# Icelk/fractal-renderer

Measured on AMD Instinct MI355X. Metric: pixel_iterations_per_sec, higher is better.
Workload: dtype f64

## Files before the change

fractal-renderer_amd/_native.py:

```python
import ctypes as C
import os

PKG_DIR = os.path.dirname(os.path.abspath(__file__))
LIB_PATH = os.path.join(PKG_DIR, "libfractal_hip.so")

FR_OK, FR_ERR_INVALID_ARGUMENT, FR_ERR_BUFFER_TOO_SMALL, FR_ERR_NO_DEVICE, FR_ERR_HIP = 0, 1, 2, 3, 4
STATUS_NAMES = {
    1: "FR_ERR_INVALID_ARGUMENT",
    2: "FR_ERR_BUFFER_TOO_SMALL",
    3: "FR_ERR_NO_DEVICE",
    4: "FR_ERR_HIP",
    5: "FR_ERR_UNSUPPORTED_ALGO",
}


class FractalHipError(RuntimeError):
    def __init__(self, code, message):
        super().__init__("%s: %s" % (STATUS_NAMES.get(code, "fr_status %d" % code), message))
        self.code = code


class Imaginary(C.Structure):

    _fields_ = [("re", C.c_double), ("im", C.c_double)]
# ... 158 lines not shown
    "fr_escape_rows": (C.c_int, [C.POINTER(fr_config), C.c_int, C.c_uint32, C.c_uint32, C.c_void_p, C.c_void_p]),
    "fr_render_rows_dd": (
        C.c_int, [C.POINTER(fr_config), C.POINTER(Imaginary), C.c_uint32, C.c_uint32, C.c_int, C.c_void_p, C.c_size_t]),
    "fr_render_rows_dd_device": (
        C.c_int,
        [C.POINTER(fr_config), C.POINTER(Imaginary), C.c_uint32, C.c_uint32, C.c_int, C.c_void_p, C.c_size_t, C.c_void_p],
    ),
    "fr_escape_rows_dd": (
        C.c_int, [C.POINTER(fr_config), C.POINTER(Imaginary), C.c_uint32, C.c_uint32, C.c_void_p, C.c_void_p]),
    "fr_render_rows_pt": (
        C.c_int, [C.POINTER(fr_config), C.POINTER(Imaginary), C.c_uint32, C.c_uint32, C.c_int, C.c_void_p, C.c_size_t]),
    "fr_render_rows_pt_device": (
        C.c_int,
        [C.POINTER(fr_config), C.POINTER(Imaginary), C.c_uint32, C.c_uint32, C.c_int, C.c_void_p, C.c_size_t, C.c_void_p],
    ),
    "fr_escape_rows_pt": (
        C.c_int, [C.POINTER(fr_config), C.POINTER(Imaginary), C.c_uint32, C.c_uint32, C.c_void_p, C.c_void_p]),
    "fr_debug_reference_orbit": (
        C.c_int, [C.POINTER(fr_config), C.POINTER(Imaginary), C.c_int, C.c_void_p, C.c_size_t, C.POINTER(C.c_uint32)]),
    "fr_colour_rgb8": (C.c_int, [C.POINTER(fr_config), C.c_void_p, C.c_void_p, C.c_size_t, C.c_void_p, C.c_size_t]),
    "fr_colour_rgb8_device": (
        C.c_int, [C.POINTER(fr_config), C.c_void_p, C.c_void_p, C.c_size_t, C.c_void_p, C.c_size_t, C.c_void_p]),
    "fr_count_iterations": (
        C.c_int,
        [C.POINTER(fr_config), C.c_int, C.c_uint32, C.c_uint32, C.c_uint32, C.c_uint32, C.POINTER(C.c_uint64),
         C.POINTER(C.c_uint64)],
    ),
    "fr_set_profiling": (C.c_int, [C.c_int]),
    "fr_last_kernel_ms": (C.c_int, [C.POINTER(C.c_float)]),
    "fr_set_tile": (C.c_int, [C.c_int]),
    "fr_set_loop_mode": (C.c_int, [C.c_int]),
    "fr_debug_loop_plan": (C.c_int, [C.POINTER(fr_config), C.c_int, C.POINTER(C.c_uint32), C.POINTER(C.c_double),
                                     C.POINTER(C.c_uint32)]),
    "fr_set_palette": (C.c_int, [C.c_int]),
    "fr_set_cycle_shortcut": (C.c_int, [C.c_int]),
    "fr_set_refill_policy": (C.c_int, [C.c_int, C.c_int]),
    "fr_debug_math": (C.c_int, [C.c_int, C.c_void_p, C.c_void_p, C.c_size_t]),
    "fr_debug_set_queue_trace": (C.c_int, [C.c_void_p]),
    "fr_debug_set_two_pass_capacity": (C.c_int, [C.c_uint32]),
}

_lib = None


def load():
    global _lib
    if _lib is not None:
        return _lib
    if not os.path.exists(LIB_PATH):
        raise ImportError(
            "%s is missing — build it first (python -c 'import __graft_entry__ as g; g.build()'); "
            "this package has no CPU fallback" % LIB_PATH
        )
    lib = C.CDLL(LIB_PATH)
    for name, (restype, argtypes) in PROTOTYPES.items():
        fn = getattr(lib, name)
        fn.restype = restype
        fn.argtypes = argtypes
    _lib = lib
    return lib


def check(rc):
    if rc != FR_OK:
        msg = load().fr_last_error()
        raise FractalHipError(rc, msg.decode() if msg else "")
# ... 1 lines not shown
```

fractal-renderer_amd/csrc/fr_api.hip:

```cpp
#include <hip/hip_runtime.h>

#include <atomic>
#include <cmath>
#include <cstddef>
#include <cstdint>
#include <cstdio>
#include <cstdlib>
#include <cstring>
#include <mutex>
#include <shared_mutex>
#include <string>
#include <vector>

#include "fr_ctx.h"

static_assert(sizeof(fr_config) == 104 && offsetof(fr_config, limit) == 16 && offsetof(fr_config, inside) == 72 &&
                  offsetof(fr_config, primary_color) == 74 && offsetof(fr_config, color_weight) == 80 &&
                  offsetof(fr_config, julia_set) == 88,
              "fr_config must stay the #[repr(C)] image of calc::Config");
static_assert(sizeof(fr_render_opts) == 32, "fr_render_opts is part of the ABI");

namespace fr {

namespace {

thread_local std::string tl_error;
thread_local Profiling tl_prof;
std::atomic<bool> g_process_exiting{false};

std::shared_mutex g_life;
std::mutex g_primary_mu;
Ctx g_primary;
bool g_primary_inited = false;

std::atomic<int> g_tile{0};
std::atomic<int> g_palette_enabled{1};
std::atomic<int> g_cycle_shortcut{0};
std::atomic<int> g_refill_minrun{-1}, g_refill_quit16{-1};
std::atomic<int> g_loop_mode{-1};
std::atomic<int> g_colour_filter{1};
std::atomic<unsigned long long *> g_queue_trace{nullptr};
std::atomic<uint32_t> g_two_pass_list_entries{0};

bool valid_tile(int tile) {
    switch (tile) {
    case 0: case 1: case 2: case 4: case 8: case 9: case 10: case 11: case 12: case 13: case 14: case 15: case 16: case 6401: case 3202: case 1604: case 808:
        return true;
    default:
        return false;
    }
}

}

int fail(int code, const char *what) {
    tl_error = what;
    return code;
}
int fail(int code, const std::string &what) {
    tl_error = what;
    return code;
}

int fail_hip(hipError_t e, const char *what) {
    char buf[512];
    snprintf(buf, sizeof buf, "%s: %s (%s)", what, hipGetErrorString(e), hipGetErrorName(e));
    tl_error = buf;
    (void)hipGetLastError();
    return (e == hipErrorNoDevice || e == hipErrorInvalidDevice) ? FR_ERR_NO_DEVICE : FR_ERR_HIP;
}

const std::string &last_error() { return tl_error; }

LifeShared::LifeShared() { g_life.lock_shared(); }
LifeShared::~LifeShared() { g_life.unlock_shared(); }
// ... 421 lines not shown
    {
        static const int dbg_want = getenv("FR_DEBUG_QUEUE_WANT") ? atoi(getenv("FR_DEBUG_QUEUE_WANT")) : 0;
        static const int dbg_minrun = getenv("FR_DEBUG_QUEUE_MINRUN") ? atoi(getenv("FR_DEBUG_QUEUE_MINRUN")) : -1;
        if (dbg_want > 0 && dbg_want <= 64) p.queue_want = (uint32_t)dbg_want;
        if (dbg_minrun >= 0) p.queue_minrun = (uint32_t)dbg_minrun;
    }
    {
        static const int dbg_ablate = getenv("FR_DEBUG_ABLATE") ? atoi(getenv("FR_DEBUG_ABLATE")) : 0;
        p.debug_ablate = (uint32_t)dbg_ablate & 3u;
    }
    p.cycle_shortcut = (o.cycle_shortcut && cfg->iterations < (1u << 30)) ? 1u : 0u;
    p.filt_k = n != 0 ? cfg->exposure / (double)n : 0.0;
    const bool filter_ok = o.colour_filter && cfg->smooth && n != 0 && std::isfinite(cfg->exposure) &&
                           std::fabs(p.filt_k) <= 1e100 && cfg->stable_limit >= 0.0;
    p.colour_filter = filter_ok ? 1u : 0u;
    const double ak = std::fabs(p.filt_k);
    p.colour_filter32 = (filter_ok && o.colour_filter == 1 && n < (1u << 24) && ak >= 0x1p-60 && ak <= 0x1p60) ? 1u : 0u;
    p.filt_k32 = (float)p.filt_k;
    p.filt_c32 = p.colour_filter32 ? std::nextafterf((float)(ak * FR_NU_BRACKET * (1.0 + 0x1p-9)), INFINITY) : 0.0f;
    for (int k = 0; k < 3; k++) {
        p.filt_d[k] = p.prim_f[k] * ak * FR_NU_BRACKET * (1.0 + 0x1p-20);
        p.filt_d32[k] = p.colour_filter32 ? std::nextafterf((float)(p.prim_f[k] * ak * FR_NU_BRACKET * (1.0 + 0x1p-10)), INFINITY) : 0.0f;
        p.prim32[k] = (float)p.prim[k];
    }
    const double lo = std::fmax(cfg->stable_limit, 2.0) * (1.0 + 0x1p-20);
    p.filt_lo32 = (p.colour_filter32 && lo < 1e30) ? std::nextafterf((float)lo, INFINITY) : INFINITY;
}

static double host_coord(double coord, double max, double offset, double pos, double scale) {
    return ((coord / max) - offset) / scale + pos;
}

constexpr uint32_t kSpecQuiet = 16;

void plan_loop(const fr_config *cfg, int precision, const Opts &o, fr_kparams &p) {
    p.loop_mode = 0;
    p.skip_t = 0.0;
    p.loop_spec = 0;
    const bool no_spec = o.loop_mode == 5;
    const int forced = no_spec ? -1 : o.loop_mode;
    if (cfg->algo != FR_ALGO_MANDELBROT && cfg->algo != FR_ALGO_JULIA) return;
    if (p.ncols == 0 || p.nrows == 0) return;
    const bool f32 = precision == FR_PRECISION_F32;
    const double range_hi = f32 ? 0x1p30 : 0x1p400;
    const double slack = f32 ? 1.0 + 0x1p-18 : 1.0 + 0x1p-30;
    double lim2;
    if (f32) {
        const float lf = (float)cfg->limit;
        lim2 = (double)(lf * lf);
    } else {
        lim2 = cfg->limit * cfg->limit;
    }
    auto mag = [f32](double v) { return std::fabs(f32 ? (double)(float)v : v); };
    const double w = (double)cfg->width, h = (double)cfg->height;
    const uint64_t x_last = (uint64_t)p.x_first + (uint64_t)(p.ncols - 1) * p.x_stride;
    const uint32_t r_last = p.nrows - 1;
    const uint64_t y_last = (uint64_t)p.y_first + (uint64_t)(r_last / p.block_rows) * p.y_stride + r_last % p.block_rows;
    if (x_last > 0xFFFFFFFFull || y_last > 0xFFFFFFFFull) return;
    auto nmax = [](double a, double b) { return (a != a || b != b) ? NAN : std::fmax(a, b); };
    double smax = 0.0;
    for (double x : {(double)p.x_first, (double)x_last})
        smax = nmax(smax, mag(host_coord(x, h, (w / h) / 2.0, cfg->pos.re, cfg->scale.re)));
    for (double y : {(double)p.y_first, (double)y_last})
        smax = nmax(smax, mag(host_coord(y, h, 0.5, cfg->pos.im, cfg->scale.im)));
    const double cmax = cfg->algo == FR_ALGO_JULIA ? nmax(mag(cfg->julia_set.re), mag(cfg->julia_set.im)) : smax;
    if (!no_spec && lim2 >= 16.0 && lim2 <= (f32 ? 0x1p100 : 0x1p1000) && cmax <= lim2 / 8.0 && smax <= (f32 ? 0x1p120 : 0x1p1000)) {
        static const int dbg = getenv("FR_DEBUG_SPEC_QUIET") ? atoi(getenv("FR_DEBUG_SPEC_QUIET")) : 0;
        p.loop_spec = dbg > 0 ? (uint32_t)dbg : kSpecQuiet;
    }
    if (forced == 0) return;
    if (!(std::fabs(cfg->limit) <= range_hi)) return;
    if (!(cmax <= range_hi)) return;
    for (int m : {4, 2}) {
        if (forced > 0 && forced != m) continue;
        double d = lim2;
        for (int j = 1; j < m && d > 0.0; j++) d = std::sqrt(d / (2.0 * slack)) - cmax;
        double t = d * (1.0 - 0x1p-20);
        if (f32) {
            float tf = (float)t;
            if ((double)tf > t) tf = std::nextafterf(tf, 0.0f);
            t = (double)tf;
        }
        if (t >= 4.5 || (forced == m && t > 0.0)) {
            p.loop_mode = (uint32_t)m;
            p.skip_t = t;
            if (!(t < lim2)) p.loop_spec = 0;
            return;
        }
    }
}

static int check_rows(const fr_config *cfg, uint32_t y0, uint32_t y1) {
    if (!cfg) return fail(FR_ERR_INVALID_ARGUMENT, "cfg is NULL");
    if (y0 > y1) return fail(FR_ERR_INVALID_ARGUMENT, "y0 > y1");
    if (y1 > cfg->height) return fail(FR_ERR_INVALID_ARGUMENT, "y1 > height");
    return FR_OK;
}

int check_precision(int precision) {
    if (precision == FR_PRECISION_DD)
        return fail(FR_ERR_INVALID_ARGUMENT, "FR_PRECISION_DD is single-device only: the row renders, fr_pixel_p, fr_escape_rows(_dd) "
                                             "and fr_count_iterations take it");
    if (precision == FR_PRECISION_PT)
        return fail(FR_ERR_INVALID_ARGUMENT, "FR_PRECISION_PT is single-device only: the row renders, fr_pixel_p, fr_escape_rows(_pt) "
                                             "and fr_count_iterations take it");
    if (precision != FR_PRECISION_F64 && precision != FR_PRECISION_F32)
        return fail(FR_ERR_INVALID_ARGUMENT, "precision must be FR_PRECISION_F64 or FR_PRECISION_F32");
    return FR_OK;
}

static int check_deep(const fr_config *cfg, const fr_imaginary *pos_lo, const char *name) {
    if (!cfg) return fail(FR_ERR_INVALID_ARGUMENT, "cfg is NULL");
    const std::string n(name);
    const double lo_re = pos_lo ? pos_lo->re : 0.0, lo_im = pos_lo ? pos_lo->im : 0.0;
    const double fields[] = {cfg->limit,    cfg->stable_limit, cfg->pos.re,       cfg->pos.im,       cfg->scale.re, cfg->scale.im,
                             cfg->exposure, cfg->color_weight, cfg->julia_set.re, cfg->julia_set.im, lo_re,         lo_im};
    for (double v : fields)
        if (!std::isfinite(v)) return fail(FR_ERR_INVALID_ARGUMENT, n + ": every field of the view must be finite");
    if (!(cfg->limit > 0.0 && cfg->limit <= 0x1p500))
// ... 995 lines not shown
}

int fr_debug_view_choice(const fr_config *cfg, int precision, uint32_t y0, uint32_t y1, int *state, int *choice,
                         uint32_t *strip_tiles) {
    if (!cfg || !state || !choice || !strip_tiles) return fail(FR_ERR_INVALID_ARGUMENT, "NULL argument");
    int rc = check_rows(cfg, y0, y1);
    if (rc == FR_OK) rc = check_precision(precision);
    if (rc != FR_OK) return rc;
    LifeShared ls;
    Ctx *ctx;
    rc = primary(&ctx);
    if (rc != FR_OK) return rc;
    fr_kparams p;
    fill_params(cfg, default_opts(), p);
    p.nrows = y1 - y0;
    p.y_first = y0;
    p.block_rows = p.nrows ? p.nrows : 1;
    p.y_stride = 0;
    const uint64_t key = view_key(cfg, p, precision);
    *state = 0, *choice = -1, *strip_tiles = 0;
    std::lock_guard<std::mutex> lk(ctx->sample_mu);
    for (int k = 0; k < Ctx::kViewChoices; k++) {
        const Ctx::ViewChoice &v = ctx->view_choices[k];
        if (v.key != key || v.state == 0) continue;
        *state = v.state;
        if (v.state == 1 && __atomic_load_n(ctx->sample_result + 8 * k + 7, __ATOMIC_ACQUIRE) == key) *state = 3;
        *choice = v.two_pass;
        *strip_tiles = v.strip_tiles;
        break;
    }
    return FR_OK;
}

int fr_debug_set_queue_trace(void *d_trace) {
    g_queue_trace.store(static_cast<unsigned long long *>(d_trace));
    return FR_OK;
}

int fr_debug_set_two_pass_capacity(uint32_t entries_per_list) {
    g_two_pass_list_entries.store(entries_per_list);
    return FR_OK;
}

int fr_debug_math(int which, const double *in, double *out, size_t n) {
    if (n == 0) return FR_OK;
    if (!in || !out) return fail(FR_ERR_INVALID_ARGUMENT, "NULL array");
    LifeShared ls;
    Ctx *ctx;
    int rc = primary(&ctx);
    if (rc != FR_OK) return rc;
    std::lock_guard<std::mutex> lk(ctx->mu);
    rc = ctx->reserve(ctx->z, 2 * n * sizeof(double));
    if (rc != FR_OK) return rc;
    double *d_in = static_cast<double *>(ctx->z.ptr), *d_out = d_in + n;
    if (which == 4) {
        if (n < 2) return fail(FR_ERR_INVALID_ARGUMENT, "which == 4 needs n >= 2");
        HIP_TRY(fr_launch_nu_scan((uint32_t)in[0], (uint32_t)in[1], d_out, ctx->stream));
        HIP_TRY(hipMemcpyAsync(out, d_out, sizeof(double), hipMemcpyDeviceToHost, ctx->stream));
        HIP_TRY(hipStreamSynchronize(ctx->stream));
        return FR_OK;
    }
    if (which == 6) {
        if (n < 2) return fail(FR_ERR_INVALID_ARGUMENT, "which == 6 needs n >= 2");
        HIP_TRY(fr_launch_cast_scan((uint32_t)in[0], (uint32_t)in[1], d_out, ctx->stream));
        unsigned long long bad = 0;
        HIP_TRY(hipMemcpyAsync(&bad, d_out, sizeof bad, hipMemcpyDeviceToHost, ctx->stream));
// ... 13 lines not shown
```

fractal-renderer_amd/csrc/fr_kernels.h:

```cpp
#ifndef FR_KERNELS_H
#define FR_KERNELS_H

#include <hip/hip_runtime.h>
#include <stdint.h>

struct fr_kparams {
    uint32_t algo;
    uint32_t width, height;
    uint32_t iterations;
    double limit, stable_limit;
    double pos_re, pos_im, scale_re, scale_im;
    double exposure;
    double julia_re, julia_im;
    uint32_t inside, smooth;
    uint32_t prim[3], sec[3];
    double prim_f[3], sec_f[3];
    double iterations_f64, inv_iterations;
    uint32_t ncols, nrows;
    uint32_t x_first, x_stride;
    uint32_t block_rows, y_first, y_stride;
    uint32_t out_in_place;
    uint32_t out_rgba;
    uint32_t loop_mode;
    double skip_t;
    uint32_t loop_spec;
    uint32_t first_no_spec;
    const uint32_t *palette;
    uint32_t palette_entries;
    uint32_t refill_minrun, refill_quit16;
    uint32_t queue_minrun, queue_want;
    uint32_t cycle_shortcut;
    uint32_t colour_filter;
    uint32_t *work_counter;
    double filt_k;
    double filt_d[3];
    uint32_t colour_filter32;
    float filt_k32;
    float filt_c32;
    float filt_d32[3];
    float prim32[3];
    float filt_lo32;
    uint32_t first_cap;
    uint32_t first_keep;
    uint32_t two_pass_cap;
    uint32_t first_only;
    uint32_t second_v1;
    uint32_t first_one_band;
    uint32_t strip_tiles;
    uint32_t debug_ablate;
    uint32_t surv_sub_capacity;
    void *surv_z;
    uint32_t *surv_pos;
    uint32_t *surv_cnt;
    void *surv_c;
    uint32_t *surv_counts;
};

constexpr uint32_t FR_SURV_QUEUES = 64;
// ... 61 lines not shown
```

fractal-renderer_amd/csrc/fr_kernels.hip:

```cpp
#include "fr_kernels.h"

#include <cmath>

#include <cstdlib>

#include "fr_math.h"

namespace {

#include "fr_colour.h"

constexpr int kWaves = 4;


#define FR_ORBIT_STEP(SFX, TAG)                    \
    "v_add_" SFX " %[t], %[r2], -%[i2]\n"          \
    "v_add_" SFX " %[x], %[re], %[re]\n"           \
    "v_add_" SFX " %[re], %[t], %[cre]\n"          \
    "v_mul_" SFX " %[x], %[x], %[im]\n"            \
    "v_add_" SFX " %[im], %[x], %[cim]\n"          \
    "v_mul_" SFX " %[r2], %[re], %[re]\n"          \
    "v_mul_" SFX " %[i2], %[im], %[im]\n"          \
    "v_add_" SFX " %[t], %[r2], %[i2]\n"           \
    "s_mov_b64 %[sprev], exec\n"                   \
// ... 167 lines not shown
    "v_mul_" SFX " %[q], %[X], %[Y]\n"             \
    "v_fma_" SFX " %[X], %[t], 0.5, %[c2re]\n"     \
    "v_add_" SFX " %[Y], %[q], %[c2im]\n"          \
    "v_mul_" SFX " %[A], %[X], %[X]\n"             \
    "v_mul_" SFX " %[B], %[Y], %[Y]\n"

#define FR_SC_IT_R(SFX, S, D)                              \
    "v_add_" SFX " %[t], %[A" S "], -%[B" S "]\n"          \
    "v_mul_" SFX " %[q], %[X" S "], %[Y" S "]\n"           \
    "v_fma_" SFX " %[X" D "], %[t], 0.5, %[c2re]\n"        \
    "v_add_" SFX " %[Y" D "], %[q], %[c2im]\n"             \
    "v_mul_" SFX " %[A" D "], %[X" D "], %[X" D "]\n"      \
    "v_mul_" SFX " %[B" D "], %[Y" D "], %[Y" D "]\n"
#define FR_SC_IT_R5(SFX, S) FR_SC_IT_R(SFX, S, S) FR_SC_IT_R(SFX, S, S) FR_SC_IT_R(SFX, S, S) FR_SC_IT_R(SFX, S, S) FR_SC_IT_R(SFX, S, S)

#define FR_SC_SPEC_ENTRY(MSTR)                                                     \
    "s_cmp_lt_u32 %[si], %[sspec]\n"                                               \
    "s_cbranch_scc1 .Lfast_%=\n"                                                   \
    "s_cmp_lt_u32 %[si], %[n]\n"                                                   \
    "s_cbranch_scc0 .Ldone_%=\n"                                                   \
    "s_sub_u32 %[stmp], %[n], %[si]\n"                                             \
    "s_cmp_ge_u32 %[stmp], " MSTR "\n"                                             \
    "s_cbranch_scc1 .Lspec_%=\n"                                                   \
    "s_mov_b32 %[sspec], %[n]\n"                                                   \
    "s_branch .Lfast_%=\n"
#define FR_SC_NOSPEC_ENTRY                                                         \
    "s_cmp_lt_u32 %[si], %[n]\n"                                                   \
    "s_cbranch_scc1 .Lfast_%=\n"                                                   \
    "s_branch .Ldone_%=\n"
#define FR_SC_SPEC_ARM                                                             \
    "s_add_u32 %[sspec], %[si], %[specq]\n"                                        \
    "s_cselect_b32 %[sspec], -1, %[sspec]\n"                                       \
    "s_min_u32 %[sspec], %[sspec], %[n]\n"
#define FR_SC_SPEC_BODY(SFX, MOV, MSTR, REST)                                      \
    ".Lspec_%=:\n" FR_SC_IT_R(SFX, "", "1") REST(SFX, "1")                         \
    "v_add_" SFX " %[t], %[A1], %[B1]\n"                                           \
    "v_cmp_nge_" SFX " vcc, %[t4lim], %[t]\n"                                      \
    "s_cbranch_vccnz .LrbA_%=\n"                                                   \
    "s_add_u32 %[si], %[si], " MSTR "\n"                                           \
    "s_sub_u32 %[stmp], %[n], %[si]\n"                                             \
    "s_cmp_ge_u32 %[stmp], " MSTR "\n"                                             \
    "s_cbranch_scc0 .LexA_%=\n"                                                    \
    FR_SC_IT_R(SFX, "1", "") REST(SFX, "")                                         \
    "v_add_" SFX " %[t], %[A], %[B]\n"                                             \
    "v_cmp_nge_" SFX " vcc, %[t4lim], %[t]\n"                                      \
    "s_cbranch_vccnz .LrbB_%=\n"                                                   \
    "s_add_u32 %[si], %[si], " MSTR "\n"                                           \
    "s_sub_u32 %[stmp], %[n], %[si]\n"                                             \
    "s_cmp_ge_u32 %[stmp], " MSTR "\n"                                             \
    "s_cbranch_scc1 .Lspec_%=\n"                                                   \
    "s_branch .Lspecout_%=\n"                                                      \
    ".LexA_%=:\n"                                                                  \
    MOV " %[X], %[X1]\n" MOV " %[Y], %[Y1]\n" MOV " %[A], %[A1]\n" MOV " %[B], %[B1]\n" \
    ".Lspecout_%=:\n"                                                              \
    "s_mov_b32 %[sspec], %[n]\n"                                                   \
    "s_cmp_lt_u32 %[si], %[n]\n"                                                   \
    "s_cbranch_scc1 .Lfast_%=\n"                                                   \
    "s_branch .Ldone_%=\n"                                                         \
    ".LrbB_%=:\n"                                                                  \
    MOV " %[X], %[X1]\n" MOV " %[Y], %[Y1]\n" MOV " %[A], %[A1]\n" MOV " %[B], %[B1]\n" \
    ".LrbA_%=:\n"                                                                  \
    "s_lshl_b32 %[specq], %[specq], 1\n"                                           \
    "s_min_u32 %[specq], %[specq], 0x8000\n"                                       \
    FR_SC_SPEC_ARM                                                                 \
    "s_branch .Lfast_%=\n"

#define FR_SC_CHECKED_STEP(SFX, TAG)               \
    FR_SC_IT(SFX)                                  \
    "v_add_" SFX " %[t], %[A], %[B]\n"             \
    "s_mov_b64 %[sprev], exec\n"                   \
    "v_cmpx_nlt_" SFX " %[lim4], %[t]\n"           \
    "s_xor_b64 %[sdiff], %[sprev], exec\n"         \
    "s_cbranch_scc1 .Lrec" TAG "_%=\n"             \
    ".Lcont" TAG "_%=:\n"

#define FR_SC_ASM(SFX, MSTR, FAST_ITS, SLOW_STEPS, SLOW_RECORDS, CYC_F, CYC_S, CYC_H, SP_INIT, SP_ARM, SP_ENTRY, SP_BODY)  \
    "s_mov_b64 %[sorig], exec\n"                                                   \
    "v_mov_b32 %[it], %[n]\n"                                                      \
    "s_mov_b32 %[si], 0\n"                                                         \
    SP_INIT                                                                        \
    "s_cbranch_execz .Ldone_%=\n"                                                  \
    "v_add_" SFX " %[t], %[A], %[B]\n"                                                         \
    "s_and_b32 %[nrem], %[n], " MSTR "-1\n"                                        \
    "s_cbranch_scc0 .Lmodesel_%=\n"                                                \
    ".Lrem_%=:\n" FR_SC_CHECKED_STEP(SFX, "R")                                     \
    "s_add_u32 %[si], %[si], 1\n"                                                  \
    "s_cmp_lt_u32 %[si], %[nrem]\n"                                                \
    "s_cbranch_scc1 .Lrem_%=\n"                                                    \
    ".Lmodesel_%=:\n"                                                              \
    "s_cmp_lt_u32 %[si], %[n]\n"                                                   \
    "s_cbranch_scc0 .Ldone_%=\n"                                                   \
    "v_cmp_lt_" SFX " vcc, %[t4lim], %[t]\n"                                       \
    "s_cbranch_vccnz .Lslow_%=\n"                                                  \
    ".Lfast_%=:\n" FAST_ITS                                                        \
// ... 53 lines not shown
    "v_mov_b32 %[vsaved], %[si]\n"                 \
    "s_lshl_b32 %[snext], %[snext], 1\n"           \
    "s_branch .Lsavecont" TAG "_%=\n"

#define FR_SC_CYC_HANDLER(TAG)                     \
    ".Lcyc" TAG "_%=:\n"                           \
    "s_or_b32 %[stmp], %[si], 0x80000000\n"        \
    "s_mov_b64 %[sprev], exec\n"                   \
    "s_mov_b64 exec, %[scyc]\n"                    \
    "v_mov_b32 %[it], %[stmp]\n"                   \
    "s_andn2_b64 exec, %[sprev], %[scyc]\n"        \
    "s_cbranch_execz .Ldone_%=\n"                  \
    "s_bcnt1_i32_b64 %[scnt], exec\n"              \
    "s_cmp_gt_u32 %[scnt], %[thr]\n"               \
    "s_cbranch_scc1 .Lcyccont" TAG "_%=\n"         \
    "s_cmp_lt_u32 %[si], %[minrun]\n"              \
    "s_cbranch_scc1 .Lcyccont" TAG "_%=\n"         \
    "s_branch .Ldone_%=\n"

#define FR_SC_ASM_M4_(SFX, CYC_F, CYC_S, CYC_H, SP_INIT, SP_ARM, SP_ENTRY, SP_BODY)                 \
    FR_SC_ASM(SFX, "4", FR_SC_IT(SFX) FR_SC_IT(SFX) FR_SC_IT(SFX) FR_SC_IT(SFX),                    \
              FR_SC_CHECKED_STEP(SFX, "A") FR_SC_CHECKED_STEP(SFX, "B") FR_SC_CHECKED_STEP(SFX, "C") \
                  FR_SC_CHECKED_STEP(SFX, "D"),                                                     \
              FR_ORBIT_RECORD("A", "0") FR_ORBIT_RECORD("B", "1") FR_ORBIT_RECORD("C", "2")         \
                  FR_ORBIT_RECORD("D", "3"),                                                        \
              CYC_F, CYC_S, CYC_H, SP_INIT, SP_ARM, SP_ENTRY, SP_BODY)
#define FR_SC_ASM_M2_(SFX, CYC_F, CYC_S, CYC_H)                                            \
    FR_SC_ASM(SFX, "2", FR_SC_IT(SFX) FR_SC_IT(SFX),                                        \
              FR_SC_CHECKED_STEP(SFX, "A") FR_SC_CHECKED_STEP(SFX, "B"),                    \
              FR_ORBIT_RECORD("A", "0") FR_ORBIT_RECORD("B", "1"), CYC_F, CYC_S, CYC_H, "", "", FR_SC_NOSPEC_ENTRY, "")
#define FR_SC_ASM_M4(SFX) FR_SC_ASM_M4_(SFX, "", "", "", "", "", FR_SC_NOSPEC_ENTRY, "")
#define FR_SC_ASM_M2(SFX) FR_SC_ASM_M2_(SFX, "", "", "")
#define FR_SC_ASM_M4_SPEC(SFX, MOV)                                                                 \
    FR_SC_ASM_M4_(SFX, "", "", "", "s_min_u32 %[sspec], %[specq], %[n]\n", FR_SC_SPEC_ARM, FR_SC_SPEC_ENTRY(FR_SPEC_MSTR), \
                  FR_SC_SPEC_BODY(SFX, MOV, FR_SPEC_MSTR, FR_SC_SPEC_REST))
#define FR_SC_CYC_HANDLERS(MOV) \
    FR_SC_CYC_HANDLER("F") FR_SC_CYC_HANDLER("S") FR_SC_CYC_SAVE(MOV, "F") FR_SC_CYC_SAVE(MOV, "S")
#define FR_SC_ASM_M4_CYC(SFX, EQ, MOV) \
    FR_SC_ASM_M4_(SFX, FR_SC_CYC_CHECK(EQ, "F"), FR_SC_CYC_CHECK(EQ, "S"), FR_SC_CYC_HANDLERS(MOV), "", "", FR_SC_NOSPEC_ENTRY, "")
#define FR_SC_ASM_M2_CYC(SFX, EQ, MOV) \
    FR_SC_ASM_M2_(SFX, FR_SC_CYC_CHECK(EQ, "F"), FR_SC_CYC_CHECK(EQ, "S"), FR_SC_CYC_HANDLERS(MOV))

template <typename T>
struct ScalableRange;
template <>
struct ScalableRange<double> {
    static constexpr double lo = 0x1p-300, hi = 0x1p400;
};
template <>
struct ScalableRange<float> {
    static constexpr float lo = 0x1p-30f, hi = 0x1p30f;
};

template <typename T>
__device__ __forceinline__ bool lane_is_scalable(T re0, T im0, T cre, T cim) {
    constexpr T lo = ScalableRange<T>::lo, hi = ScalableRange<T>::hi;
    auto c_ok = [=](T v) { return __builtin_fabs(v) >= lo && __builtin_fabs(v) <= hi; };
    auto s_ok = [=](T v) { return v == (T)0 || c_ok(v); };
    return c_ok(cre) && c_ok(cim) && s_ok(re0) && s_ok(im0);
}

template <typename T, int M, bool CYC>
__device__ __forceinline__ uint32_t orbit_scaled_run(uint32_t iterations, T &X, T &Y, T &A, T &B, T c2re, T c2im,
                                                     T squared, T skip_t, EpisodeCtl ctl, uint32_t &completed,
                                                     T *pXs = nullptr, T *pYs = nullptr,
                                                     uint32_t *saved_index = nullptr, uint32_t spec_quiet = 0u) {
    uint32_t it;
    T t, q;
    T X1, Y1, A1, B1;
    uint32_t sspec;
    uint32_t specq = __builtin_amdgcn_readfirstlane(spec_quiet ? spec_quiet : 0xFFFFFFFFu);
    T Xs = CYC ? *pXs : T(0), Ys = CYC ? *pYs : T(0);
    uint32_t vsaved = 0xFFFFFFFFu;
    uint32_t snext = 32u;
    unsigned long long sorig, sprev, sdiff, scyc;
    uint32_t si, stmp, nrem, scnt;
    const uint32_t n = __builtin_amdgcn_readfirstlane(iterations);
    const uint32_t thr = __builtin_amdgcn_readfirstlane(ctl.thr), minrun = __builtin_amdgcn_readfirstlane(ctl.minrun);
    const T lim4_v = (T)4 * squared, t4_v = (T)4 * skip_t;
#define FR_SC_OUTPUTS                                                                                           \
    [X] "+v"(X), [Y] "+v"(Y), [A] "+v"(A), [B] "+v"(B), [it] "=&v"(it), [t] "=&v"(t), [q] "=&v"(q),             \
        [sorig] "=&s"(sorig), [sprev] "=&s"(sprev), [sdiff] "=&s"(sdiff), [si] "=&s"(si), [stmp] "=&s"(stmp),   \
        [nrem] "=&s"(nrem), [scnt] "=&s"(scnt)
#define FR_SC_INPUTS                                                                                            \
    [c2re] "v"(c2re), [c2im] "v"(c2im), [lim4] "s"(lim4), [t4lim] "s"(t4lim), [n] "s"(n), [thr] "s"(thr),       \
        [minrun] "s"(minrun)
#define FR_SC_OPERANDS : FR_SC_OUTPUTS : FR_SC_INPUTS : "vcc", "scc"
#define FR_SC_OPERANDS_SPEC                                                                                     \
    : FR_SC_OUTPUTS, [X1] "=&v"(X1), [Y1] "=&v"(Y1), [A1] "=&v"(A1), [B1] "=&v"(B1), [sspec] "=&s"(sspec),      \
      [specq] "+&s"(specq)                                                                                      \
    : FR_SC_INPUTS                                                                                              \
    : "vcc", "scc"
#define FR_SC_OPERANDS_CYC                                                                                      \
    : FR_SC_OUTPUTS, [scyc] "=&s"(scyc), [Xs] "+v"(Xs), [Ys] "+v"(Ys), [vsaved] "+v"(vsaved), [snext] "+s"(snext) \
    : FR_SC_INPUTS                                                                                              \
    : "vcc", "scc"
    if constexpr (sizeof(T) == 8) {
        const uint64_t lb = fr_bits_of(lim4_v), tb = fr_bits_of(t4_v);
        const uint64_t lim4 = (uint64_t)(uint32_t)__builtin_amdgcn_readfirstlane((uint32_t)lb) |
                              ((uint64_t)(uint32_t)__builtin_amdgcn_readfirstlane((uint32_t)(lb >> 32)) << 32);
        const uint64_t t4lim = (uint64_t)(uint32_t)__builtin_amdgcn_readfirstlane((uint32_t)tb) |
                               ((uint64_t)(uint32_t)__builtin_amdgcn_readfirstlane((uint32_t)(tb >> 32)) << 32);
        if constexpr (M == 4 && CYC)
            asm volatile(FR_SC_ASM_M4_CYC("f64", "v_cmp_eq_u64", "v_mov_b64") FR_SC_OPERANDS_CYC);
        else if constexpr (M == 4)
            asm volatile(FR_SC_ASM_M4_SPEC("f64", "v_mov_b64") FR_SC_OPERANDS_SPEC);
        else if constexpr (CYC)
            asm volatile(FR_SC_ASM_M2_CYC("f64", "v_cmp_eq_u64", "v_mov_b64") FR_SC_OPERANDS_CYC);
        else
            asm volatile(FR_SC_ASM_M2("f64") FR_SC_OPERANDS);
    } else {
        const uint32_t lim4 = __builtin_amdgcn_readfirstlane(__builtin_bit_cast(uint32_t, lim4_v));
        const uint32_t t4lim = __builtin_amdgcn_readfirstlane(__builtin_bit_cast(uint32_t, t4_v));
        if constexpr (M == 4 && CYC)
            asm volatile(FR_SC_ASM_M4_CYC("f32", "v_cmp_eq_u32", "v_mov_b32") FR_SC_OPERANDS_CYC);
        else if constexpr (M == 4)
            asm volatile(FR_SC_ASM_M4_SPEC("f32", "v_mov_b32") FR_SC_OPERANDS_SPEC);
        else if constexpr (CYC)
            asm volatile(FR_SC_ASM_M2_CYC("f32", "v_cmp_eq_u32", "v_mov_b32") FR_SC_OPERANDS_CYC);
        else
            asm volatile(FR_SC_ASM_M2("f32") FR_SC_OPERANDS);
    }
    (void)scyc;
    (void)snext;
    (void)X1, (void)Y1, (void)A1, (void)B1, (void)sspec, (void)specq;
    if constexpr (CYC) {
        *pXs = Xs;
        *pYs = Ys;
        *saved_index = vsaved;
    }
    completed = si;
    return it;
}

template <typename T, int M>
__device__ __forceinline__ uint32_t orbit_scaled(uint32_t iterations, T &re, T &im, T cre, T cim, T squared,
                                                 T skip_t, T &r2, T &i2, uint32_t spec_quiet = 0u) {
    T X = re + re, Y = im + im, A = X * X, B = Y * Y;
    uint32_t completed;
    const uint32_t it = orbit_scaled_run<T, M, false>(iterations, X, Y, A, B, cre + cre, cim + cim, squared, skip_t,
                                               EpisodeCtl{0, 0}, completed, nullptr, nullptr, nullptr, spec_quiet);
    re = X * (T)0.5;
    im = Y * (T)0.5;
    r2 = re * re;
    i2 = im * im;
    return it;
}

template <typename T>
__device__ __forceinline__ uint32_t orbit_auto(uint32_t loop_mode, uint32_t iterations, T &re, T &im, T cre, T cim,
                                               T squared, T skip_t, T &r2, T &i2, int strip_scalable = -1,
                                               uint32_t spec_quiet = 0u) {
    if (loop_mode != 0 && strip_scalable != 0) {
        bool all_ok = strip_scalable == 1;
        if (strip_scalable < 0) all_ok = __ballot(!lane_is_scalable<T>(re, im, cre, cim)) == 0ull;
        if (all_ok) {
            if (loop_mode == 4) return orbit_scaled<T, 4>(iterations, re, im, cre, cim, squared, skip_t, r2, i2, spec_quiet);
            return orbit_scaled<T, 2>(iterations, re, im, cre, cim, squared, skip_t, r2, i2);
        }
    }
    return orbit<T>(iterations, re, im, cre, cim, squared, r2, i2, spec_quiet);
}

__device__ __forceinline__ double coord_to_space(double coord, double max, double offset, double pos,
                                                 double scale) {
    return ((coord / max) - offset) / scale + pos;
}

__device__ __forceinline__ void store_pixel(uint32_t ncols, uint32_t out_rgba, uint8_t *base, uint32_t row, uint32_t col,
                                            const uint8_t rgb[3]) {
    const uint64_t k = (uint64_t)row * ncols + col;
    if (out_rgba) {
        reinterpret_cast<uint32_t *>(base)[k] =
            (uint32_t)rgb[0] | ((uint32_t)rgb[1] << 8) | ((uint32_t)rgb[2] << 16) | 0xFF000000u;
    } else {
        uint8_t *o = base + 3ull * k;
        o[0] = rgb[0];
        o[1] = rgb[1];
        o[2] = rgb[2];
    }
}
__device__ __forceinline__ void store_pixel(const fr_kparams &p, uint8_t *base, uint32_t row, uint32_t col, const uint8_t rgb[3]) {
    store_pixel(p.ncols, p.out_rgba, base, row, col, rgb);
}

typedef const __attribute__((address_space(4))) fr_kparams *KArgs;
#define FR_COLD_PARAMS(NAME)                                                          \
    KArgs NAME = (KArgs)__builtin_amdgcn_kernarg_segment_ptr();  \
    asm volatile("" : "+s"(NAME))

// ... 20 lines not shown

__device__ __forceinline__ void store_packed(uint8_t *base, uint32_t off, uint32_t packed, uint32_t bpp) {
    if (bpp == 4u) {
        const uint32_t v = packed | 0xFF000000u;
        asm volatile("s_nop 4\n\tglobal_store_dword %0, %1, %2" : : "v"(off), "v"(v), "s"(base) : "memory");
    } else {
        asm volatile("s_nop 4\n\tglobal_store_short %0, %1, %2\n\tglobal_store_byte_d16_hi %0, %1, %2 offset:2" : : "v"(off), "v"(packed), "s"(base) : "memory");
    }
}

struct TileOut {
    uint8_t *base;
    uint32_t lane_off, bpp;
    bool narrow, fast_colour;
};

template <typename T>
__device__ __forceinline__ uint32_t colour_packed(bool valid, bool fast_colour, T re, T im, T r2, T i2, uint32_t iters,
                                                  const double *lds_tab, const uint32_t *palette) {
    uint32_t packed = 0;
    unsigned long long todo = ballot64(valid);
    if (fast_colour) {
        Filter32 f;
        {
            FR_COLD_PARAMS(kp);
            f.lo = kp->filt_lo32, f.k = kp->filt_k32, f.c = kp->filt_c32;
            f.p0 = kp->prim32[0], f.p1 = kp->prim32[2], f.p2 = kp->prim32[1];
        }
        float d32;
        if constexpr (sizeof(T) == 8)
            d32 = (float)(r2 + i2);
        else
            d32 = r2 + i2;
        uint32_t pk;
        const bool decided = colour_fast32(f, d32, (float)(iters + 1u), pk);
        const bool ok = valid && d32 >= f.lo && d32 <= 0x1.ffffep119f && decided;
        packed = ok ? pk : 0u;
        todo &= ~ballot64(ok);
    }
    if (todo != 0ull) {
        bool inside_done = false;
        if (lane_in(todo)) {
            double dist;
            if constexpr (sizeof(T) == 8) {
                dist = (double)(r2 + i2);
            } else {
                const double zre = (double)re, zim = (double)im;
                dist = zre * zre + zim * zim;
            }
            FR_COLD_PARAMS(kp);
            inside_done = !(dist > kp->stable_limit);
            if (inside_done && kp->inside)
                packed = sat_u8_dev(kp->sec_f[0] * dist) | (sat_u8_dev(kp->sec_f[2] * dist) << 8) | (sat_u8_dev(kp->sec_f[1] * dist) << 16);
        }
        todo &= ~ballot64(inside_done);
    }
    if (todo != 0ull) {
        if (lane_in(todo)) {
            FR_COLD_PARAMS(kp);
            const ColourConsts cc = make_colour_consts(*kp);
            uint8_t rgb[3];
            colour_pixel<T>(cc, re, im, r2, i2, iters, lds_tab, palette, rgb);
            packed = (uint32_t)rgb[0] | ((uint32_t)rgb[1] << 8) | ((uint32_t)rgb[2] << 16);
        }
    }
    return packed;
}

template <typename T, int MODE>
__device__ __forceinline__ void render_pixel(const fr_kparams &p, const fr_kout &out, const double *s_tab,
                                             const uint32_t *s_pal, double sre, double sim, bool valid,
                                             uint32_t cx, uint32_t r, uint32_t lane, uint32_t r_out,
                                             int strip_scalable = -1, const TileOut *to = nullptr) {
    double zre = 0.0, zim = 0.0;
    T tre = 0, tim = 0, tr2 = 0, ti2 = 0;
    uint32_t iters = 0;
    const bool escape_algo = p.algo == 0  || p.algo == 2 ;
    if (valid && escape_algo) {
        const double cre = p.algo == 0 ? sre : p.julia_re;
        const double cim = p.algo == 0 ? sim : p.julia_im;
        if constexpr (sizeof(T) == 8) {
            tre = sre;
            tim = sim;
            iters = orbit_auto<double>(p.loop_mode, p.iterations, tre, tim, cre, cim, p.limit * p.limit, p.skip_t,
                                       tr2, ti2, strip_scalable, p.loop_spec);
            zre = tre;
            zim = tim;
        } else {
            tre = (float)sre, tim = (float)sim;
            const float lim = (float)p.limit;
            iters = orbit_auto<float>(p.loop_mode, p.iterations, tre, tim, (float)cre, (float)cim, lim * lim,
                                      (float)p.skip_t, tr2, ti2, strip_scalable, p.loop_spec);
            zre = (double)tre;
            zim = (double)tim;
        }
    }

    if constexpr (MODE == FR_OUT_RGB) {
        if (to != nullptr) {
            uint32_t packed = 0;
            if (escape_algo) packed = colour_packed<T>(valid, to->fast_colour, tre, tim, tr2, ti2, iters, s_tab, s_pal);
            if (valid) {
                if (to->narrow) {
                    store_packed(to->base, to->lane_off, packed, to->bpp);
                } else {
                    const uint8_t rgb[3] = {(uint8_t)packed, (uint8_t)(packed >> 8), (uint8_t)(packed >> 16)};
                    store_pixel(p, out.rgb, r_out, cx, rgb);
                }
            }
        } else if (valid) {
            uint8_t rgb[3] = {0, 0, 0};
            if (escape_algo) {
                const ColourConsts cc = make_colour_consts(p);
                colour_pixel<T>(cc, tre, tim, tr2, ti2, iters, s_tab, s_pal, rgb);
            }
            store_pixel(p, out.rgb, r_out, cx, rgb);
        }
    } else if constexpr (MODE == FR_OUT_ESCAPE) {
        if (valid) {
            const uint64_t k = (uint64_t)r * p.ncols + cx;
            if (out.z) {
                out.z[2 * k] = zre;
                out.z[2 * k + 1] = zim;
            }
            if (out.iters) out.iters[k] = iters;
// ... 1005 lines not shown
            const uint32_t cx = tile0 * 8u + ccol, r = row0 + crow;
            if (cx < p.ncols && r < p.nrows) {
                const T zre = (T)sre, zim = (T)sim;
                const T cre = julia ? (T)p.julia_re : zre, cim = julia ? (T)p.julia_im : zim;
                if constexpr (FORM == 0) {
                    a0 = zre, a1 = zim, a2 = zre * zre, a3 = zim * zim, c0 = cre, c1 = cim;
                } else {
                    a0 = zre + zre, a1 = zim + zim, a2 = a0 * a0, a3 = a1 * a1, c0 = cre + cre, c1 = cim + cim;
                }
                if constexpr (CYC) xs = ys = cycle_none<T>(), saved_at = 0;
                px = cx, py = r, pout = sout;
                done = 0;
                busy = true;
            }
        }
        const uint32_t nfree = (uint32_t)__builtin_popcountll(free_mask);
        next = next + nfree < P ? next + nfree : P;
        const unsigned long long busy_mask = __ballot(busy);
        if (busy_mask == 0ull) {
            if (next >= P) break;
            continue;
        }

        const uint32_t n = wave_min_u32(busy ? iterations - done : 0xFFFFFFFFu);
        const uint32_t nbusy = (uint32_t)__builtin_popcountll(busy_mask);
        EpisodeCtl ctl{0u, 0u};
        if (next < P) ctl = EpisodeCtl{nbusy - (nbusy * p.refill_quit16 + 15) / 16, p.refill_minrun};
        uint32_t it = 0, completed = 0, saved_index = 0xFFFFFFFFu;
        if (busy) {
            if constexpr (FORM == 0)
                it = orbit_run<T>(n, a0, a1, c0, c1, squared, a2, a3, ctl, completed, p.loop_spec);
            else
                it = orbit_scaled_run<T, FORM, CYC>(n, a0, a1, a2, a3, c0, c1, squared, skip_t, ctl, completed, &xs, &ys,
                                                    &saved_index, p.loop_spec);
        }
        if (busy) {
            bool cycled = false;
            if constexpr (CYC) cycled = (it & 0x80000000u) != 0u;
            const bool escaped = !cycled && it < completed;
            const uint32_t before = done;
            if constexpr (CYC) {
                if (saved_index != 0xFFFFFFFFu) saved_at = before + saved_index;
            }
            if (cycled) {
                const uint32_t k = it & 0x7FFFFFFFu;
                const uint32_t d = before + k - saved_at;
                const uint32_t remaining = iterations - (before + k);
                done = iterations - remaining % d;
                xs = ys = cycle_none<T>();
            } else {
                done += completed;
            }
            if (escaped || done == iterations) {
                const uint32_t iters = escaped ? before + it : iterations;
                T fre, fim, fr2, fi2;
                if constexpr (FORM == 0) {
                    fre = a0, fim = a1, fr2 = a2, fi2 = a3;
                } else {
                    fre = a0 * (T)0.5, fim = a1 * (T)0.5;
                    fr2 = fre * fre, fi2 = fim * fim;
                }
                const double zre = (double)fre, zim = (double)fim;
                const double dist = sizeof(T) == 8 ? (double)(fr2 + fi2) : zre * zre + zim * zim;
                if constexpr (MODE == FR_OUT_RGB) {
                    uint8_t rgb[3];
                    colour_of(cc, dist, iters, s_tab, s_pal, rgb);
                    store_pixel(p, out.rgb, pout, px, rgb);
// ... 1475 lines not shown
```

include/fractal_hip.h:

```cpp
#ifndef FRACTAL_HIP_H
#define FRACTAL_HIP_H

#include <stddef.h>
#include <stdint.h>

#ifdef __cplusplus
extern "C" {
#endif

#define FR_ABI_VERSION 3

typedef enum fr_status {
    FR_OK = 0,
    FR_ERR_INVALID_ARGUMENT = 1,
    FR_ERR_BUFFER_TOO_SMALL = 2,
    FR_ERR_NO_DEVICE = 3,
    FR_ERR_HIP = 4,
    FR_ERR_UNSUPPORTED_ALGO = 5
} fr_status;

typedef enum fr_algo {
    FR_ALGO_MANDELBROT = 0,
    FR_ALGO_BARNSLEY_FERN = 1,
    FR_ALGO_JULIA = 2
// ... 166 lines not shown
int fr_escape_rows(const fr_config *cfg, int precision, uint32_t y0, uint32_t y1, double *z_re_im,
                   uint32_t *iters);

int fr_colour_rgb8(const fr_config *cfg, const double *z_re_im, const uint32_t *iters, size_t n, uint8_t *out,
                   size_t out_len);
int fr_colour_rgb8_device(const fr_config *cfg, const void *d_z_re_im, const void *d_iters, size_t n, void *d_out,
                          size_t out_len, void *hip_stream);


int fr_count_iterations(const fr_config *cfg, int precision, uint32_t y0, uint32_t y1, uint32_t sx,
                        uint32_t sy, uint64_t *total, uint64_t *pixels);

int fr_set_profiling(int enabled);
int fr_last_kernel_ms(float *ms);
int fr_last_kernel_name(char *buf, size_t buf_len);

int fr_set_tile(int tile);

int fr_set_dispatch_sampling(int enabled);
int fr_debug_sample_view(const fr_config *cfg, int precision, double out[8]);
int fr_debug_view_choice(const fr_config *cfg, int precision, uint32_t y0, uint32_t y1, int *state, int *choice,
                         uint32_t *strip_tiles);

int fr_set_refill_policy(int minrun, int quit16);

int fr_set_cycle_shortcut(int enabled);

int fr_set_palette(int enabled);

int fr_set_colour_filter(int enabled);

int fr_set_loop_mode(int mode);
int fr_debug_loop_plan(const fr_config *cfg, int precision, uint32_t *loop_mode, double *skip_t, uint32_t *spec_quiet);

int fr_debug_math(int which, const double *in, double *out, size_t n);
int fr_debug_set_queue_trace(void *d_trace);
int fr_debug_set_two_pass_capacity(uint32_t entries_per_list);

#ifdef __cplusplus
}
#endif
#endif
```

Before: 5312 billion.

## Grow speculative escape-check blocks geometrically up to a capped length

The speculative Mandelbrot/Julia inner loop checked for escape every fixed block of iterations. It now doubles the block length after each block without an escape, up to a cap (default 128, with a debug setter). On rollback the cap is reset to the base block. Fewer escape checks and branches run per iteration in long non-escaping stretches, at the cost of more rolled-back iterations when a lane escapes late in a long block. The colour filter is also gated on a wave ballot so fast-colour work is skipped when no lane is outside.

```diff
diff --git a/fractal-renderer_amd/_native.py b/fractal-renderer_amd/_native.py
--- a/fractal-renderer_amd/_native.py
+++ b/fractal-renderer_amd/_native.py
@@ -214,6 +214,8 @@
     "fr_set_loop_mode": (C.c_int, [C.c_int]),
     "fr_debug_loop_plan": (C.c_int, [C.POINTER(fr_config), C.c_int, C.POINTER(C.c_uint32), C.POINTER(C.c_double),
                                      C.POINTER(C.c_uint32)]),
+    "fr_debug_set_spec_maxlen": (C.c_int, [C.c_uint32]),
+    "fr_debug_spec_maxlen": (C.c_int, [C.POINTER(fr_config), C.c_int, C.POINTER(C.c_uint32)]),
     "fr_set_palette": (C.c_int, [C.c_int]),
     "fr_set_cycle_shortcut": (C.c_int, [C.c_int]),
     "fr_set_refill_policy": (C.c_int, [C.c_int, C.c_int]),
diff --git a/fractal-renderer_amd/csrc/fr_api.hip b/fractal-renderer_amd/csrc/fr_api.hip
--- a/fractal-renderer_amd/csrc/fr_api.hip
+++ b/fractal-renderer_amd/csrc/fr_api.hip
@@ -41,6 +41,7 @@
 std::atomic<int> g_colour_filter{1};
 std::atomic<unsigned long long *> g_queue_trace{nullptr};
 std::atomic<uint32_t> g_two_pass_list_entries{0};
+std::atomic<uint32_t> g_spec_maxlen{0};
 
 bool valid_tile(int tile) {
     switch (tile) {
@@ -528,11 +529,20 @@
 }
 
 constexpr uint32_t kSpecQuiet = 16;
+constexpr uint32_t kSpecBlock = 16, kSpecMaxLen = 128;
+
+static uint32_t spec_maxlen() {
+    const uint32_t asked = g_spec_maxlen.load(), want = asked ? asked : kSpecMaxLen;
+    uint32_t len = kSpecBlock;
+    while (len < 0x8000u && 2u * len <= want) len *= 2u;
+    return len;
+}
 
 void plan_loop(const fr_config *cfg, int precision, const Opts &o, fr_kparams &p) {
     p.loop_mode = 0;
     p.skip_t = 0.0;
     p.loop_spec = 0;
+    p.loop_spec_max = 0;
     const bool no_spec = o.loop_mode == 5;
     const int forced = no_spec ? -1 : o.loop_mode;
     if (cfg->algo != FR_ALGO_MANDELBROT && cfg->algo != FR_ALGO_JULIA) return;
@@ -563,6 +573,7 @@
     if (!no_spec && lim2 >= 16.0 && lim2 <= (f32 ? 0x1p100 : 0x1p1000) && cmax <= lim2 / 8.0 && smax <= (f32 ? 0x1p120 : 0x1p1000)) {
         static const int dbg = getenv("FR_DEBUG_SPEC_QUIET") ? atoi(getenv("FR_DEBUG_SPEC_QUIET")) : 0;
         p.loop_spec = dbg > 0 ? (uint32_t)dbg : kSpecQuiet;
+        p.loop_spec_max = spec_maxlen();
     }
     if (forced == 0) return;
     if (!(std::fabs(cfg->limit) <= range_hi)) return;
@@ -580,7 +591,7 @@
         if (t >= 4.5 || (forced == m && t > 0.0)) {
             p.loop_mode = (uint32_t)m;
             p.skip_t = t;
-            if (!(t < lim2)) p.loop_spec = 0;
+            if (!(t < lim2)) p.loop_spec = p.loop_spec_max = 0;
             return;
         }
     }
@@ -1642,6 +1653,26 @@
     return FR_OK;
 }
 
+int fr_debug_set_spec_maxlen(uint32_t maxlen) {
+    g_spec_maxlen.store(maxlen);
+    return FR_OK;
+}
+
+int fr_debug_spec_maxlen(const fr_config *cfg, int precision, uint32_t *maxlen) {
+    if (!cfg || !maxlen) return fail(FR_ERR_INVALID_ARGUMENT, "NULL argument");
+    int rc = check_precision(precision);
+    if (rc != FR_OK) return rc;
+    const Opts o = default_opts();
+    fr_kparams p;
+    fill_params(cfg, o, p);
+    p.nrows = cfg->height;
+    p.block_rows = cfg->height ? cfg->height : 1;
+    p.y_stride = 0;
+    plan_loop(cfg, precision, o, p);
+    *maxlen = p.loop_spec_max;
+    return FR_OK;
+}
+
 int fr_debug_set_queue_trace(void *d_trace) {
     g_queue_trace.store(static_cast<unsigned long long *>(d_trace));
     return FR_OK;
diff --git a/fractal-renderer_amd/csrc/fr_kernels.h b/fractal-renderer_amd/csrc/fr_kernels.h
--- a/fractal-renderer_amd/csrc/fr_kernels.h
+++ b/fractal-renderer_amd/csrc/fr_kernels.h
@@ -24,6 +24,7 @@
     uint32_t loop_mode;
     double skip_t;
     uint32_t loop_spec;
+    uint32_t loop_spec_max;
     uint32_t first_no_spec;
     const uint32_t *palette;
     uint32_t palette_entries;
diff --git a/fractal-renderer_amd/csrc/fr_kernels.hip b/fractal-renderer_amd/csrc/fr_kernels.hip
--- a/fractal-renderer_amd/csrc/fr_kernels.hip
+++ b/fractal-renderer_amd/csrc/fr_kernels.hip
@@ -223,24 +223,35 @@
     "s_add_u32 %[sspec], %[si], %[specq]\n"                                        \
     "s_cselect_b32 %[sspec], -1, %[sspec]\n"                                       \
     "s_min_u32 %[sspec], %[sspec], %[n]\n"
+#define FR_SC_SPEC_BLOCK(SFX, MSTR, REST, TAG, S, D, RB, NEXT, EXIT)               \
+    ".Lblk" TAG "_%=:\n" FR_SC_IT_R(SFX, S, D)                                     \
+    "s_mov_b32 %[stmp], %[nrem]\n"                                                 \
+    ".Lmid" TAG "_%=:\n" REST(SFX, D)                                              \
+    "s_sub_u32 %[stmp], %[stmp], " MSTR "\n"                                       \
+    "s_cmp_lt_u32 %[stmp], " MSTR "\n"                                             \
+    "s_cbranch_scc1 .Ltst" TAG "_%=\n"                                             \
+    FR_SC_IT_R(SFX, D, D)                                                          \
+    "s_branch .Lmid" TAG "_%=\n"                                                   \
+    ".Ltst" TAG "_%=:\n"                                                           \
+    "v_add_" SFX " %[t], %[A" D "], %[B" D "]\n"                                   \
+    "v_cmp_nge_" SFX " vcc, %[t4lim], %[t]\n"                                      \
+    "s_cbranch_vccnz " RB "\n"                                                     \
+    "s_add_u32 %[si], %[si], %[nrem]\n"                                            \
+    "s_lshl_b32 %[nrem], %[nrem], 1\n"                                             \
+    "s_min_u32 %[nrem], %[nrem], %[lcap]\n"                                        \
+    "s_sub_u32 %[stmp], %[n], %[si]\n"                                             \
+    ".Lfit" TAG "_%=:\n"                                                           \
+    "s_cmp_le_u32 %[nrem], %[stmp]\n"                                              \
+    "s_cbranch_scc1 " NEXT "\n"                                                    \
+    "s_lshr_b32 %[nrem], %[nrem], 1\n"                                             \
+    "s_cmp_ge_u32 %[nrem], " MSTR "\n"                                             \
+    "s_cbranch_scc1 .Lfit" TAG "_%=\n"                                             \
+    "s_branch " EXIT "\n"
 #define FR_SC_SPEC_BODY(SFX, MOV, MSTR, REST)                                      \
-    ".Lspec_%=:\n" FR_SC_IT_R(SFX, "", "1") REST(SFX, "1")                         \
-    "v_add_" SFX " %[t], %[A1], %[B1]\n"                                           \
-    "v_cmp_nge_" SFX " vcc, %[t4lim], %[t]\n"                                      \
-    "s_cbranch_vccnz .LrbA_%=\n"                                                   \
-    "s_add_u32 %[si], %[si], " MSTR "\n"                                           \
-    "s_sub_u32 %[stmp], %[n], %[si]\n"                                             \
-    "s_cmp_ge_u32 %[stmp], " MSTR "\n"                                             \
-    "s_cbranch_scc0 .LexA_%=\n"                                                    \
-    FR_SC_IT_R(SFX, "1", "") REST(SFX, "")                                         \
-    "v_add_" SFX " %[t], %[A], %[B]\n"                                             \
-    "v_cmp_nge_" SFX " vcc, %[t4lim], %[t]\n"                                      \
-    "s_cbranch_vccnz .LrbB_%=\n"                                                   \
-    "s_add_u32 %[si], %[si], " MSTR "\n"                                           \
-    "s_sub_u32 %[stmp], %[n], %[si]\n"                                             \
-    "s_cmp_ge_u32 %[stmp], " MSTR "\n"                                             \
-    "s_cbranch_scc1 .Lspec_%=\n"                                                   \
-    "s_branch .Lspecout_%=\n"                                                      \
+    ".Lspec_%=:\n"                                                                 \
+    "s_mov_b32 %[nrem], " MSTR "\n"                                                \
+    FR_SC_SPEC_BLOCK(SFX, MSTR, REST, "A", "", "1", ".LrbA_%=", ".LblkB_%=", ".LexA_%=") \
+    FR_SC_SPEC_BLOCK(SFX, MSTR, REST, "B", "1", "", ".LrbB_%=", ".LblkA_%=", ".Lspecout_%=") \
     ".LexA_%=:\n"                                                                  \
     MOV " %[X], %[X1]\n" MOV " %[Y], %[Y1]\n" MOV " %[A], %[A1]\n" MOV " %[B], %[B1]\n" \
     ".Lspecout_%=:\n"                                                              \
@@ -251,6 +262,7 @@
     ".LrbB_%=:\n"                                                                  \
     MOV " %[X], %[X1]\n" MOV " %[Y], %[Y1]\n" MOV " %[A], %[A1]\n" MOV " %[B], %[B1]\n" \
     ".LrbA_%=:\n"                                                                  \
+    "s_mov_b32 %[lcap], " MSTR "\n"                                                \
     "s_lshl_b32 %[specq], %[specq], 1\n"                                           \
     "s_min_u32 %[specq], %[specq], 0x8000\n"                                       \
     FR_SC_SPEC_ARM                                                                 \
@@ -370,7 +382,7 @@
 #define FR_SC_ASM_M4(SFX) FR_SC_ASM_M4_(SFX, "", "", "", "", "", FR_SC_NOSPEC_ENTRY, "")
 #define FR_SC_ASM_M2(SFX) FR_SC_ASM_M2_(SFX, "", "", "")
 #define FR_SC_ASM_M4_SPEC(SFX, MOV)                                                                 \
-    FR_SC_ASM_M4_(SFX, "", "", "", "s_min_u32 %[sspec], %[specq], %[n]\n", FR_SC_SPEC_ARM, FR_SC_SPEC_ENTRY(FR_SPEC_MSTR), \
+    FR_SC_ASM_M4_(SFX, "", "", "", "s_min_u32 %[sspec], %[specq], %[n]\n" "s_max_u32 %[lcap], %[lcap], " FR_SPEC_MSTR "\n", FR_SC_SPEC_ARM, FR_SC_SPEC_ENTRY(FR_SPEC_MSTR), \
                   FR_SC_SPEC_BODY(SFX, MOV, FR_SPEC_MSTR, FR_SC_SPEC_REST))
 #define FR_SC_CYC_HANDLERS(MOV) \
     FR_SC_CYC_HANDLER("F") FR_SC_CYC_HANDLER("S") FR_SC_CYC_SAVE(MOV, "F") FR_SC_CYC_SAVE(MOV, "S")
@@ -402,12 +414,14 @@
 __device__ __forceinline__ uint32_t orbit_scaled_run(uint32_t iterations, T &X, T &Y, T &A, T &B, T c2re, T c2im,
                                                      T squared, T skip_t, EpisodeCtl ctl, uint32_t &completed,
                                                      T *pXs = nullptr, T *pYs = nullptr,
-                                                     uint32_t *saved_index = nullptr, uint32_t spec_quiet = 0u) {
+                                                     uint32_t *saved_index = nullptr, uint32_t spec_quiet = 0u,
+                                                     uint32_t spec_maxlen = 0u) {
     uint32_t it;
     T t, q;
     T X1, Y1, A1, B1;
     uint32_t sspec;
     uint32_t specq = __builtin_amdgcn_readfirstlane(spec_quiet ? spec_quiet : 0xFFFFFFFFu);
+    uint32_t lcap = __builtin_amdgcn_readfirstlane(spec_maxlen);
     T Xs = CYC ? *pXs : T(0), Ys = CYC ? *pYs : T(0);
     uint32_t vsaved = 0xFFFFFFFFu;
     uint32_t snext = 32u;
@@ -426,7 +440,7 @@
 #define FR_SC_OPERANDS : FR_SC_OUTPUTS : FR_SC_INPUTS : "vcc", "scc"
 #define FR_SC_OPERANDS_SPEC                                                                                     \
     : FR_SC_OUTPUTS, [X1] "=&v"(X1), [Y1] "=&v"(Y1), [A1] "=&v"(A1), [B1] "=&v"(B1), [sspec] "=&s"(sspec),      \
-      [specq] "+&s"(specq)                                                                                      \
+      [specq] "+&s"(specq), [lcap] "+&s"(lcap)                                                                  \
     : FR_SC_INPUTS                                                                                              \
     : "vcc", "scc"
 #define FR_SC_OPERANDS_CYC                                                                                      \
@@ -461,7 +475,7 @@
     }
     (void)scyc;
     (void)snext;
-    (void)X1, (void)Y1, (void)A1, (void)B1, (void)sspec, (void)specq;
+    (void)X1, (void)Y1, (void)A1, (void)B1, (void)sspec, (void)specq, (void)lcap;
     if constexpr (CYC) {
         *pXs = Xs;
         *pYs = Ys;
@@ -473,11 +487,11 @@
 
 template <typename T, int M>
 __device__ __forceinline__ uint32_t orbit_scaled(uint32_t iterations, T &re, T &im, T cre, T cim, T squared,
-                                                 T skip_t, T &r2, T &i2, uint32_t spec_quiet = 0u) {
+                                                 T skip_t, T &r2, T &i2, uint32_t spec_quiet = 0u, uint32_t spec_maxlen = 0u) {
     T X = re + re, Y = im + im, A = X * X, B = Y * Y;
     uint32_t completed;
     const uint32_t it = orbit_scaled_run<T, M, false>(iterations, X, Y, A, B, cre + cre, cim + cim, squared, skip_t,
-                                               EpisodeCtl{0, 0}, completed, nullptr, nullptr, nullptr, spec_quiet);
+                                               EpisodeCtl{0, 0}, completed, nullptr, nullptr, nullptr, spec_quiet, spec_maxlen);
     re = X * (T)0.5;
     im = Y * (T)0.5;
     r2 = re * re;
@@ -488,12 +502,12 @@
 template <typename T>
 __device__ __forceinline__ uint32_t orbit_auto(uint32_t loop_mode, uint32_t iterations, T &re, T &im, T cre, T cim,
                                                T squared, T skip_t, T &r2, T &i2, int strip_scalable = -1,
-                                               uint32_t spec_quiet = 0u) {
+                                               uint32_t spec_quiet = 0u, uint32_t spec_maxlen = 0u) {
     if (loop_mode != 0 && strip_scalable != 0) {
         bool all_ok = strip_scalable == 1;
         if (strip_scalable < 0) all_ok = __ballot(!lane_is_scalable<T>(re, im, cre, cim)) == 0ull;
         if (all_ok) {
-            if (loop_mode == 4) return orbit_scaled<T, 4>(iterations, re, im, cre, cim, squared, skip_t, r2, i2, spec_quiet);
+            if (loop_mode == 4) return orbit_scaled<T, 4>(iterations, re, im, cre, cim, squared, skip_t, r2, i2, spec_quiet, spec_maxlen);
             return orbit_scaled<T, 2>(iterations, re, im, cre, cim, squared, skip_t, r2, i2);
         }
     }
@@ -580,11 +594,14 @@
             d32 = (float)(r2 + i2);
         else
             d32 = r2 + i2;
-        uint32_t pk;
-        const bool decided = colour_fast32(f, d32, (float)(iters + 1u), pk);
-        const bool ok = valid && d32 >= f.lo && d32 <= 0x1.ffffep119f && decided;
-        packed = ok ? pk : 0u;
-        todo &= ~ballot64(ok);
+        const unsigned long long outside = ballot64(valid && d32 >= f.lo);
+        if (outside != 0ull) {
+            uint32_t pk;
+            const bool decided = colour_fast32(f, d32, (float)(iters + 1u), pk);
+            const bool ok = lane_in(outside) && d32 <= 0x1.ffffep119f && decided;
+            packed = ok ? pk : 0u;
+            todo &= ~ballot64(ok);
+        }
     }
     if (todo != 0ull) {
         bool inside_done = false;
@@ -631,14 +648,14 @@
             tre = sre;
             tim = sim;
             iters = orbit_auto<double>(p.loop_mode, p.iterations, tre, tim, cre, cim, p.limit * p.limit, p.skip_t,
-                                       tr2, ti2, strip_scalable, p.loop_spec);
+                                       tr2, ti2, strip_scalable, p.loop_spec, p.loop_spec_max);
             zre = tre;
             zim = tim;
         } else {
             tre = (float)sre, tim = (float)sim;
             const float lim = (float)p.limit;
             iters = orbit_auto<float>(p.loop_mode, p.iterations, tre, tim, (float)cre, (float)cim, lim * lim,
-                                      (float)p.skip_t, tr2, ti2, strip_scalable, p.loop_spec);
+                                      (float)p.skip_t, tr2, ti2, strip_scalable, p.loop_spec, p.loop_spec_max);
             zre = (double)tre;
             zim = (double)tim;
         }
@@ -1710,7 +1727,7 @@
                 it = orbit_run<T>(n, a0, a1, c0, c1, squared, a2, a3, ctl, completed, p.loop_spec);
             else
                 it = orbit_scaled_run<T, FORM, CYC>(n, a0, a1, a2, a3, c0, c1, squared, skip_t, ctl, completed, &xs, &ys,
-                                                    &saved_index, p.loop_spec);
+                                                    &saved_index, p.loop_spec, p.loop_spec_max);
         }
         if (busy) {
             bool cycled = false;
diff --git a/include/fractal_hip.h b/include/fractal_hip.h
--- a/include/fractal_hip.h
+++ b/include/fractal_hip.h
@@ -222,6 +222,8 @@
 
 int fr_set_loop_mode(int mode);
 int fr_debug_loop_plan(const fr_config *cfg, int precision, uint32_t *loop_mode, double *skip_t, uint32_t *spec_quiet);
+int fr_debug_set_spec_maxlen(uint32_t maxlen);
+int fr_debug_spec_maxlen(const fr_config *cfg, int precision, uint32_t *maxlen);
 
 int fr_debug_math(int which, const double *in, double *out, size_t n);
 int fr_debug_set_queue_trace(void *d_trace);
```

New measurement: 5427 billion (median of 6 runs). 1.02x the previous value.
